# phylo42/IPK

Hardware: AMD Instinct MI355X
Metric: scored phylo-k-mers/sec (higher is better)
Workload: dtype f32

## Files before the change

ipk_amd/csrc/ipkgpu.hip:

```cpp
#include <cstring>
#include <hip/hip_runtime.h>
#include <rocprim/rocprim.hpp>

#include <algorithm>
#include <cmath>
#include <cstdarg>
#include <cstdio>
#include <cstring>
#include <new>
#include <string>
#include <type_traits>
#include <unordered_map>
#include <memory>
#include <vector>

#include "../../include/ipkgpu.h"
#include "dcla_device.hpp"
#include "kernels_score.hpp"
#include "kernels_quad.hpp"
#include "kernels_compact.hpp"
#include "kernels_keymajor.hpp"
#include "kernels_reduce_pipe.hpp"
#include "kernels_filter.hpp"
#include "kernels_dbfile.hpp"
// ... 59 lines not shown
    ipkgpu_comm* comm = nullptr;
    hipStream_t stream = nullptr;
    std::string err;
    int64_t workspace_bytes = 0;
    int64_t opt_variant = 0;
    int64_t opt_flags = 0;
    int64_t opt_kmc_pass = 0;
    int64_t opt_slice = 0;
    uint64_t sliced_windows = 0;
    int64_t opt_prefix_mats = 0;
    int64_t opt_wg_chunks2 = 0;
    int64_t opt_rounds = 0;
    int64_t opt_pool_limit = 0;
    int64_t opt_pool_chunks = 0;
    DevBuf table, best, ovfq, counts, offsets, goff, idx, branch, scan_sums, scan_boff, tmp_a, tmp_b, tmp_c;
    DevBuf pool, desc, gbcnt, gboff, gbcur, clist, gm, tile_next;
    DevBuf ptrs;
    DevBuf sp_bits, sp_pops, sp_rank, sp_c16;
    void* h_spill[2] = {nullptr, nullptr}; hipEvent_t ev_spill[2] = {nullptr, nullptr}; size_t h_spill_cap = 0;
    size_t held = 0, held_peak = 0;
    int64_t budget = 0;
    size_t refused_need = 0;
    DevBuf mask;
    bool mask_valid = false;
    uint64_t mask_words = 0;
    bool table_compressed = false;
    DevBuf rank, vaddr, ucnt, qpack, xstart, pcounts;
    DevBuf seq, pvals, pvaddr, mrank, cursnap;
    DevBuf cvals, coff, croom;
    bool comp_own_vals = false;
// ... 234 lines not shown
        *got = ctx->free_blocks[best].second;
        ctx->live_blocks[*out] = *got;
        ctx->cached_bytes -= *got;
        ctx->free_blocks.erase(ctx->free_blocks.begin() + best);
        return hipSuccess;
    }
    const hipError_t e = ctx_alloc(ctx, out, want_bytes);
    if (e == hipSuccess) *got = ctx->live_blocks[*out];
    return e;
}

static std::vector<DevBuf*> all_workspaces(ipkgpu_ctx* ctx)
{
    return {&ctx->table, &ctx->best, &ctx->ovfq, &ctx->counts, &ctx->offsets, &ctx->goff, &ctx->idx,
            &ctx->branch, &ctx->scan_sums, &ctx->scan_boff, &ctx->tmp_a, &ctx->tmp_b, &ctx->tmp_c,
            &ctx->pool, &ctx->desc, &ctx->gbcnt, &ctx->gboff, &ctx->gbcur, &ctx->clist, &ctx->gm, &ctx->tile_next, &ctx->mask,
            &ctx->rank, &ctx->vaddr, &ctx->ucnt, &ctx->qpack, &ctx->xstart, &ctx->pcounts, &ctx->ptrs,
            &ctx->cvals, &ctx->coff, &ctx->croom, &ctx->seq, &ctx->pvals, &ctx->pvaddr, &ctx->mrank, &ctx->cursnap,
            &ctx->sp_bits, &ctx->sp_pops, &ctx->sp_rank, &ctx->sp_c16,
            &ctx->place_seq, &ctx->place_off, &ctx->place_out, &ctx->place_tables, &ctx->place_small, &ctx->place_amb};
}

extern "C" {

uint32_t ipkgpu_bits_per_symbol(uint32_t sigma) { return sigma == 4 ? 2u : sigma == 20 ? 5u : 0u; }
uint32_t ipkgpu_max_k(uint32_t sigma) { return sigma == 4 ? 14u : sigma == 20 ? 6u : 0u; }
uint32_t ipkgpu_max_k_keyrange(uint32_t sigma) { return sigma == 4 ? 16u : ipkgpu_max_k(sigma); }
size_t ipkgpu_kmer_batch(uint32_t key, size_t n_ranges) { return n_ranges ? key % n_ranges : 0; }

float ipkgpu_log_threshold(float omega, uint32_t sigma, uint32_t k)
{
// ... 324 lines not shown
#ifndef IPK_QROWLANE
#define IPK_QROWLANE 0
#endif
template <int SIGMA, int K> constexpr bool quad_rowlane() { return K <= 10 ? IPK_QROWLANE != 0 : IPK_QROWLANE12 != 0; }
#ifndef IPK_QONEWIN12
#define IPK_QONEWIN12 1
#endif
template <int SIGMA, int K> constexpr bool quad_onewin() { return K >= 11 && IPK_QONEWIN12 != 0 && quad_rowlane<SIGMA, K>(); }
#ifndef IPK_PAIR6
#define IPK_PAIR6 1
#endif
template <int SIGMA, int K> constexpr PairLayout quad_layout()
{
    return IPK_PAIR6 != 0 && quad_ok<SIGMA, K>() && K <= 10 && !quad_rowlane<SIGMA, K>() ? PairLayout::PAIR6 : PairLayout::PAIR8;
}
template <int SIGMA, int K> size_t quad_lds()
{
    if constexpr (!quad_ok<SIGMA, K>()) return 0;
    else {
        constexpr int CAP = fast_cap<SIGMA, K>();
        constexpr uint32_t TBL = stream_tbl<SIGMA, K>();
        constexpr uint32_t NB = (uint32_t)((ipow(SIGMA, K) + TBL - 1) / TBL);
        return QuadTile<SIGMA, K, quad_tw<SIGMA, K>()>::HEAD_BYTES + (size_t)quad_nw<SIGMA, K>() * quad_wave_entries<SIGMA, K, CAP, quad_onewin<SIGMA, K>()>() * 8 +
               (size_t)quad_nw<SIGMA, K>() * NB * 8;
    }
}
template <int SIGMA, int K, bool COUNT_ONLY = false>
int launch_quad_pass1(ipkgpu_ctx* ctx, const StreamParams& sp, uint32_t n_wg, PairLayout layout)
{
    if constexpr (!quad_ok<SIGMA, K>()) { (void)sp; (void)n_wg; (void)layout; return fail(ctx, IPKGPU_ERR_INVALID, "quad kernel unsupported for this sigma/k"); }
    else {
        if (layout != quad_layout<SIGMA, K>()) return fail(ctx, IPKGPU_ERR_INVALID, "the pass' pool layout is not the quad kernel's");
        constexpr int CAP = fast_cap<SIGMA, K>();
        constexpr uint32_t TBL = stream_tbl<SIGMA, K>();
        constexpr int QNW = quad_nw<SIGMA, K>(), QTW = quad_tw<SIGMA, K>();
        const size_t lds = quad_lds<SIGMA, K>();
        auto kern = score_quad_kernel<SIGMA, K, CAP, QTW, QNW, TBL, COUNT_ONLY, quad_rowlane<SIGMA, K>(), quad_onewin<SIGMA, K>(), quad_layout<SIGMA, K>()>;
        if (lds > 64 * 1024)
            HIP_TRY(ctx, hipFuncSetAttribute(reinterpret_cast<const void*>(kern), hipFuncAttributeMaxDynamicSharedMemorySize, (int)lds));
        hipLaunchKernelGGL(kern, dim3(n_wg), dim3(QNW * 64), lds, ctx->stream, sp);
        HIP_TRY(ctx, hipGetLastError());
        return IPKGPU_OK;
    }
}

#ifndef IPK_XPNW
#define IPK_XPNW 11
#endif
#ifndef IPK_XPTW
#define IPK_XPTW 128
#endif
constexpr int XP_TW = IPK_XPTW;
// ... 123 lines not shown
            case 15 * 8 + 2: return f(int_c<4>{}, int_c<15>{}, int_c<13>{});
            case 16 * 8 + 2: return f(int_c<4>{}, int_c<16>{}, int_c<14>{});
            case 16 * 8 + 3: return f(int_c<4>{}, int_c<16>{}, int_c<13>{});
        }
    }
    return fail(ctx, IPKGPU_ERR_INVALID, "unsupported key range");
}

struct Geometry {
    uint32_t fast_cap = 0;
    uint32_t stream_nb = 0, stream_tbl = 0;
    uint32_t stream_nw = NW, stream_tw = TW;
    size_t stream_lds = 0;
    bool quad = false;
    uint32_t quad_nw = NW, quad_tw = TW;
    size_t quad_lds = 0;
    PairLayout quad_layout = PairLayout::PAIR8;
    uint32_t xp_nb = 0, xp_tbl = 0;
    size_t xp_lds = 0;
};

int fill_geometry(ipkgpu_ctx* ctx, uint32_t sigma, uint32_t k, uint32_t lead, Geometry& g)
{
    if (!lead)
        RC_TRY(with_sigma_k(ctx, sigma, k, [&](auto S_, auto K_) {
            g.fast_cap = fast_cap<S_, K_>();
            g.stream_nb = stream_nb<S_, K_>(); g.stream_tbl = stream_tbl<S_, K_>();
            g.stream_nw = stream_nw<S_, K_>(); g.stream_tw = stream_tw<S_, K_>(); g.stream_lds = stream_lds<S_, K_>();
            g.quad = quad_ok<S_, K_>();
            g.quad_nw = quad_nw<S_, K_>(); g.quad_tw = quad_tw<S_, K_>(); g.quad_lds = quad_lds<S_, K_>();
            g.quad_layout = quad_layout<S_, K_>();
            return IPKGPU_OK;
        }));
    return with_xp_shape(ctx, sigma, k, lead, [&](auto S_, auto K_, auto KK_) {
        g.xp_nb = xp_nb<S_, K_, KK_>(); g.xp_tbl = xp_tbl<S_, K_>(); g.xp_lds = xp_lds<S_, K_, KK_>();
        return IPKGPU_OK;
    });
}

#ifndef IPK_KMC_RUNS_DEFAULT
#define IPK_KMC_RUNS_DEFAULT 1
#endif
#ifndef IPK_KMC_PASS
#define IPK_KMC_PASS 256
#endif
#define KM_LAUNCH(KERN, CAPV, ...)                                                                                        \
// ... 486 lines not shown
        else if (cap < n_waves * NBK * SUB) {
            if (gb > 1) return IPKGPU_RETRY_SMALLER;
            return fail(ctx, IPKGPU_ERR_NOMEM, "the pair pool of ONE branch group does not fit device memory");
        }
        RC_TRY(ensure(ctx, ctx->pool, (cap + 1) * CHB));
        RC_TRY(ensure(ctx, ctx->desc, cap * 8));
        if (!forced) cap = std::min<uint64_t>(ctx->pool.cap / CHB - 1, ctx->desc.cap / 8);
        RC_TRY(ensure(ctx, ctx->gbcnt, 2 * n_gb * 4));
        uint32_t* const d_gbcur = ctx->gbcnt.as<uint32_t>() + n_gb;
        RC_TRY(ensure(ctx, ctx->gboff, (n_gb + 1) * 8));
        uint32_t* d_pool_next = small_at(ctx, SMALL_POOL_NEXT);
        uint32_t* d_pool_ovf = small_at(ctx, SMALL_POOL_OVF);
        const bool pre_ok = use_quad && n_waves * NBK + 1024 <= cap && !(ctx->opt_flags & 32);
        const uint32_t pre_chunks = pre_ok ? (uint32_t)(n_waves * NBK) : 0u;
        uint32_t* d_tile_next = nullptr;
        if (use_quad && !(ctx->opt_flags & 128) && ((uint64_t)nb * s_tiles_per_mat >= 4ull * gb * S || (ctx->opt_flags & 256))) {
            RC_TRY(ensure(ctx, ctx->tile_next, (size_t)gb * 4));
            d_tile_next = ctx->tile_next.as<uint32_t>();
        }
        hipLaunchKernelGGL(small_reset_kernel, dim3((std::max<uint32_t>(gb, SMALL_XP_TOO_BIG / 4) + 255) / 256), dim3(256), 0, ctx->stream,
                           reinterpret_cast<uint32_t*>(ctx->small), pre_chunks, d_tile_next, gb, S);
        HIP_TRY(ctx, hipGetLastError());
        HIP_TRY(ctx, hipMemsetAsync(ctx->desc.p, 0, cap * 8, ctx->stream));

        StreamParams sp;
        sp.logp = logp_dev; sp.best = ctx->best.as<float>();
        sp.gm_off = ctx->gm.as<uint32_t>(); sp.gm_list = ctx->gm.as<uint32_t>() + gb + 1;
        sp.sites = pl.sites; sp.nwin = pl.nwin; sp.tiles_per_mat = s_tiles_per_mat; sp.S = S;
        sp.eps = pl.eps;
        sp.pool = ctx->pool.as<uint2>(); sp.pool_cap = (uint32_t)cap; sp.pool_next = d_pool_next;
        sp.desc = ctx->desc.as<unsigned long long>(); sp.pool_ovf = d_pool_ovf;
        sp.emitted = p.emitted; sp.ovf_queue = p.ovf_queue; sp.ovf_count = p.ovf_count; sp.mat_slot = p.mat_slot;
        sp.flags = (uint32_t)(ctx->opt_flags);
        sp.pre_chunks = pre_chunks;
        sp.tile_next = d_tile_next;
        std::unique_ptr<Stopwatch> sw_own(new Stopwatch(ctx->stream, &ctx->events));
        Stopwatch& sw = *sw_own;
        const int ev_a = sw.mark();
        RC_TRY(pass1(sp, n_wg, false));
        const int ev_b = sw.mark();
        const bool spec = ctx->spec_skip_wait && !s_compress && !(ctx->opt_flags & 64);
        uint32_t n_ovf = 0;
        uint32_t h[2] = {0, 0};
        if (!spec) {
            HIP_TRY(ctx, hipMemcpyAsync(ctx->h_rb, ctx->small, SMALL_BYTES, hipMemcpyDeviceToHost, ctx->stream));
            HIP_TRY(ctx, hipStreamSynchronize(ctx->stream));
            n_ovf = ctx->h_rb[SMALL_OVF_COUNT / 4]; h[0] = ctx->h_rb[SMALL_POOL_NEXT / 4]; h[1] = ctx->h_rb[SMALL_POOL_OVF / 4];
        }
        const bool ovf_in_pool = n_ovf > 0 && ((uint64_t)n_ovf * IPK_OVF_POOL_RATIO >= windows || s_compress) && pool_ovf_ok;
        if (ovf_in_pool) {
// ... 1469 lines not shown
extern "C" {

int ipkgpu_get_option(const ipkgpu_ctx* ctx, const char* name, int64_t* value)
{
    if (!ctx || !name || !value) return IPKGPU_ERR_INVALID;
    if (!strcmp(name, "workspace_bytes")) { *value = ctx->workspace_bytes; return IPKGPU_OK; }
    if (!strcmp(name, "device_budget_bytes")) { *value = ctx->budget; return IPKGPU_OK; }
    if (!strcmp(name, "last_refused_bytes")) { *value = (int64_t)ctx->refused_need; return IPKGPU_OK; }
    if (!strcmp(name, "slice_long_lists")) { *value = ctx->opt_slice; return IPKGPU_OK; }
    if (!strcmp(name, "db_load_chunk_bytes")) { *value = ctx->opt_load_chunk; return IPKGPU_OK; }
    if (!strcmp(name, "place_batch_queries")) { *value = ctx->opt_place_batch; return IPKGPU_OK; }
    if (!strcmp(name, "place_lds_branches")) { *value = ctx->opt_place_lds; return IPKGPU_OK; }
    if (!strcmp(name, "debug_sliced_windows")) { *value = (int64_t)ctx->sliced_windows; return IPKGPU_OK; }
    if (!strcmp(name, "debug_count_pass_pairs")) { *value = (int64_t)ctx->count_pass_pairs; return IPKGPU_OK; }
    if (!strcmp(name, "debug_count_pass_queued")) { *value = (int64_t)ctx->count_pass_queued; return IPKGPU_OK; }
    if (!strcmp(name, "debug_pool_bytes")) { *value = (int64_t)ctx->pool.cap; return IPKGPU_OK; }
    return IPKGPU_ERR_INVALID;
}

int ipkgpu_mem_stats(ipkgpu_ctx* ctx, uint64_t* held, uint64_t* held_peak, int reset_peak)
{
    if (!ctx) return IPKGPU_ERR_INVALID;
    if (held) *held = ctx->held;
    if (held_peak) *held_peak = ctx->held_peak;
    if (reset_peak) ctx->held_peak = ctx->held;
    return IPKGPU_OK;
}

int ipkgpu_parts_spill(ipkgpu_ctx* ctx, ipkgpu_parts* parts, const char* dir, uint32_t piece, uint64_t* bytes_written)
{
// ... 201 lines not shown
```

ipk_amd/csrc/kernels_quad.hpp:

```cpp
#pragma once
#include "kernels_score.hpp"

namespace ipkgpu {

struct QuadNode { int J, H, TH, OFF; uint32_t F, CMUL; };
struct QuadStep { int H, A, B; };

template <int SIGMA, int K>
struct QuadGeo {
    using D = HalvesDD<SIGMA, K>;
    static constexpr int HL = D::HL, HR = D::HR, LA = D::LA, LB = D::LB, RA = D::RA, RB = D::RB;
    static constexpr bool OK = SIGMA == 4 && D::OK && LA >= 2 && LA <= 3 && LB >= 2 && LB <= 3 && RA >= 2 && RA <= 3 && RB >= 2 && RB <= 3;
    static constexpr uint32_t FLA = D::FLA, FLB = D::FLB, FRA = D::FRA, FRB = D::FRB;
    static constexpr uint32_t mulR = ipow(SIGMA, K - K / 2);
    static constexpr uint32_t CW = FLA + FLB + FRA + FRB;
    static constexpr int th_n(int h) { return h == 2 ? 3 : 5; }
    static constexpr int TH0 = 2, TH1 = TH0 + th_n(LA), TH2 = TH1 + th_n(LB), TH3 = TH2 + th_n(RA);
    static constexpr int TH_F = TH3 + th_n(RB);
    static constexpr int PADW = 1;
    static constexpr QuadNode node(int n)
    {
        return n == 0 ? QuadNode{0, LA, TH0, 0, FLA, 1u}
             : n == 1 ? QuadNode{LA, LB, TH1, (int)FLA, FLB, mulR}
             : n == 2 ? QuadNode{HL, RA, TH2, (int)(FLA + FLB), FRA, 1u}
                      : QuadNode{HL + RA, RB, TH3, (int)(FLA + FLB + FRA), FRB, 1u};
    }
    static constexpr int count_h(int h) { int c = 0; for (int n = 0; n < 4; ++n) c += node(n).H == h; return c; }
    static constexpr int nth_h(int h, int i) { for (int n = 0; n < 4; ++n) if (node(n).H == h) { if (i == 0) return n; --i; } return -1; }
    static constexpr int NS2 = (count_h(2) + 1) / 2, NS3 = (count_h(3) + 1) / 2, NSTEPS = NS2 + NS3;
    static constexpr QuadStep step(int s)
    {
        return s < NS2 ? QuadStep{2, nth_h(2, 2 * s), nth_h(2, 2 * s + 1)} : QuadStep{3, nth_h(3, 2 * (s - NS2)), nth_h(3, 2 * (s - NS2) + 1)};
    }
    static constexpr int step_of(int n) { for (int s = 0; s < NSTEPS; ++s) if (step(s).A == n || step(s).B == n) return s; return -1; }
    static constexpr int slot_of(int n) { return step(step_of(n)).B == n ? 1 : 0; }
    static constexpr int NS1 = (count_h(2) > 0 ? 1 : 0) + (count_h(3) > 0 ? 1 : 0);
    static constexpr int step1_h(int s) { return (s == 0 && count_h(2) > 0) ? 2 : 3; }
    static constexpr int step1_node(int s, int slot) { return nth_h(step1_h(s), slot); }
    static constexpr int step1_of(int n) { return node(n).H == 2 ? 0 : (count_h(2) > 0 ? 1 : 0); }
    static constexpr int slot1_of(int n) { int c = 0; for (int m = 0; m < n; ++m) c += node(m).H == node(n).H; return c; }
};

template <int SIGMA, int K, int TW>
struct QuadTile {
    static constexpr int TC = TW + K - 1 + QuadGeo<SIGMA, K>::PADW;
    static constexpr int COLS_F = TC * SIGMA;
    static constexpr int BEST_F = ((TC + 1 + 3) / 4) * 4;
    static constexpr int TH_FLOATS = (((TW + QuadGeo<SIGMA, K>::PADW) * QuadGeo<SIGMA, K>::TH_F + 3) / 4) * 4;
    static constexpr int HEAD_BYTES = (COLS_F + BEST_F + TH_FLOATS) * 4;
};

template <int SIGMA, int K, int CAP, bool ONEWIN = false>
constexpr uint32_t quad_wave_entries()
{
    using Q = QuadGeo<SIGMA, K>;
    return (ONEWIN ? 1 : 2) * Q::CW + Geo<SIGMA, Q::HL, CAP>::CAPH + Geo<SIGMA, Q::HR, CAP>::CAPH;
}

template <int J, int H>
__device__ __forceinline__ void quad_node_thresholds(const float* bs, float e, float* out)
{
    out[0] = e;
    if constexpr (H == 2) {
        out[1] = e - (bs[J + 2] - bs[J + 1]);
        out[2] = e - (bs[J + 1] - bs[J]);
// ... 30 lines not shown
__device__ __forceinline__ uint2 lds_entry(uint32_t base, uint32_t j)
{
    typedef const u32x2_t __attribute__((address_space(3)))* lds_pair_ptr;
    uint32_t a;
    asm("v_lshl_add_u32 %0, %1, 3, %2" : "=v"(a) : "v"(j), "s"(base));
    const u32x2_t v = *(lds_pair_ptr)(uintptr_t)a;
    return make_uint2(v.x, v.y);
}
__device__ __forceinline__ uint32_t bcnt_add(uint32_t x, uint32_t acc)
{
    uint32_t r;
    asm("v_bcnt_u32_b32 %0, %1, %2" : "=v"(r) : "v"(x), "v"(acc));
    return r;
}

template <int H>
__device__ __forceinline__ void quad_step(const float* ca, const float* cb, const float* ci, uint64_t vmask, const float* th, uint32_t list,
                                          uint32_t sh16, uint32_t lt16, uint32_t lt16w, uint32_t code16, uint32_t cmul, uint32_t& count)
{
    const float e = th[0];
    if constexpr (H == 2) {
        const float sl = ca[0], sr = cb[0];
        const float s = sl + sr;
        const bool c1 = sl > th[1], c2 = sr > th[2], c3 = s > e;
        const uint64_t m = vmask & ballot64(c1) & ballot64(c2) & ballot64(c3);
        const uint32_t x = (uint32_t)(m >> sh16);
        lds_put8_lanes(lshl3_add((uint32_t)__popc(x & lt16), list), code16, __float_as_uint(s), m);
        count = (uint32_t)__popc(x & 0xFFFFu);
    } else {
        const float sj = ca[0], sl2 = cb[0];
        const float s2 = sj + sl2;
        const bool d1 = sj > th[3], d2 = sl2 > th[4], d3 = s2 > th[2];
        const uint64_t mp = vmask & ballot64(d1) & ballot64(d2) & ballot64(d3);
        float s[4]; uint64_t m[4]; uint32_t x[4];
#pragma unroll
        for (int i = 0; i < 4; ++i) {
            const float si = ci[i];
            s[i] = si + s2;
            const bool c1 = si > th[1], c2 = s[i] > e;
            m[i] = mp & ballot64(c1) & ballot64(c2);
            x[i] = (uint32_t)(m[i] >> sh16);
        }
        const uint32_t y01 = __builtin_amdgcn_perm(x[1], x[0], 0x05040100u);
        const uint32_t y23 = __builtin_amdgcn_perm(x[3], x[2], 0x05040100u);
        const uint32_t n01 = (uint32_t)__popc(y01);
        const uint32_t pos[4] = {(uint32_t)__popc(x[0] & lt16), (uint32_t)__popc(y01 & lt16w), bcnt_add(x[2] & lt16, n01), bcnt_add(y23 & lt16w, n01)};
#pragma unroll
        for (int i = 0; i < 4; ++i) lds_put8_lanes(lshl3_add(pos[i], list), __umul24(cmul, (uint32_t)i * 16u) + code16, __float_as_uint(s[i]), m[i]);
        count = bcnt_add(y23, n01);
    }
}

__device__ __forceinline__ void pool_store(uint2* wave_base, uint32_t byte_off, uint2 val)
{
    const unsigned long long data = ((unsigned long long)val.y << 32) | val.x;
    asm volatile("global_store_dwordx2 %0, %1, %2" : : "v"(byte_off), "v"(data), "s"(wave_base) : "memory");
}
__device__ __forceinline__ void pool_store_lanes(uint2* wave_base, uint32_t byte_off, uint2 val, uint64_t mask)
{
    const unsigned long long data = ((unsigned long long)val.y << 32) | val.x;
    IPK_ASSERT_FULL_EXEC();
    asm volatile("s_mov_b64 exec, %3\n\tglobal_store_dwordx2 %0, %1, %2\n\ts_mov_b64 exec, -1"
                 : : "v"(byte_off), "v"(data), "s"(wave_base), "s"(mask) : "memory");
// ... 32 lines not shown
__device__ __forceinline__ uint64_t pool_store_inside6(uint2* wave_base, uint32_t off4, uint32_t off2, uint2 val, uint32_t v, uint64_t pass, uint32_t CH)
{
    static_assert(SLOT_PLANE < 4096, "the slot plane's offset must fit the store's immediate field");
    uint64_t outside;
    IPK_ASSERT_FULL_EXEC();
    asm volatile("s_mov_b64 exec, %7\n\t"
                 "v_cmpx_gt_u32_e32 vcc, %8, %6\n\t"
                 "global_store_dword %1, %3, %5\n\t"
                 "global_store_short %2, %4, %5 offset:%9\n\t"
                 "s_andn2_b64 %0, %7, exec\n\t"
                 "s_mov_b64 exec, -1"
                 : "=&s"(outside) : "v"(off4), "v"(off2), "v"(val.y), "v"(val.x), "s"(wave_base), "v"(v), "s"(pass), "s"(CH), "n"(SLOT_PLANE)
                 : "memory", "vcc");
    return outside;
}

constexpr uint32_t QUAD_SPAN_BYTES_LOG2 = 32;
constexpr uint32_t QUAD_SPAN_TEST = 8;

__device__ __forceinline__ uint32_t div_small(float x_plus_half, float rn) { return (uint32_t)(x_plus_half * rn); }

template <uint32_t NB, uint32_t CH, uint32_t PAIR_BYTES = 8u>
struct RowAppender {
    static constexpr uint32_t NONE = 0xFFFFFFFFu;
    static constexpr uint32_t CHUNK_BYTES = CH * PAIR_BYTES;
    static constexpr uint32_t SPAN_CHUNKS = (uint32_t)((1ull << QUAD_SPAN_BYTES_LOG2) / CHUNK_BYTES);
    const StreamParams& p;
    unsigned long long* st;
    uint32_t g;
    uint32_t chunk_next = 0, chunk_end = 0;
// ... 151 lines not shown
    uint32_t n = 0;
    for (uint32_t i0 = 0; i0 < na; i0 += rps) {
        const uint2 a = ap[i0];
        const float s = __uint_as_float(a.y) + by;
        const bool live = lane < min(rps, na - i0) * nb, c = s > eps;
        const uint64_t m = ballot64(live) & ballot64(c);
        const uint32_t cnt = (uint32_t)__popcll(m);
        if (n + cnt > cap) return LIST_OVERFLOW;
        if (live && c) (out + n)[mbcnt(m)] = make_uint2(a.x * MUL + b.x, __float_as_uint(s));
        n += cnt;
    }
    return n;
}

template <int SIGMA, int K, int CAP, int TW, int NW, uint32_t TBL, bool COUNT_ONLY = false, bool ROWLANE = false, bool ONEWIN = false,
          PairLayout LAYOUT = PairLayout::PAIR8>
__global__ __launch_bounds__(NW * 64) void score_quad_kernel(StreamParams p)
{
    extern __shared__ __align__(16) unsigned char smem[];
    using Q = QuadGeo<SIGMA, K>;
    using QT = QuadTile<SIGMA, K, TW>;
    static_assert(Q::OK, "quad kernel: DNA k = 8..12");
    constexpr uint32_t T = ipow(SIGMA, K);
    constexpr uint32_t NB = (T + TBL - 1) / TBL;
    constexpr uint32_t CH = chunk_pairs<TBL>();
    constexpr uint32_t mulR = Q::mulR;
    static_assert(TBL % mulR == 0, "a row of the final join must stay inside one bucket");
    using CL = ChunkLayout<TBL, LAYOUT>;
    static_assert(!ROWLANE || LAYOUT == PairLayout::PAIR8, "the row-per-lane join writes 8-byte pairs");
    constexpr bool P6 = LAYOUT == PairLayout::PAIR6;
    constexpr uint32_t CAPL = Geo<SIGMA, Q::HL, CAP>::CAPH, CAPR = Geo<SIGMA, Q::HR, CAP>::CAPH;
    constexpr uint32_t WS = quad_wave_entries<SIGMA, K, CAP, ONEWIN>();
    constexpr uint32_t WPW = ONEWIN ? 1u : 2u;
    constexpr int NST = ONEWIN ? Q::NS1 : Q::NSTEPS;
    float* cols = reinterpret_cast<float*>(smem);
    float* best = cols + QT::COLS_F;
    float* thr = best + QT::BEST_F;
    uint2* scratch_all = reinterpret_cast<uint2*>(smem + QT::HEAD_BYTES);
    unsigned long long* state_all = reinterpret_cast<unsigned long long*>(scratch_all + (size_t)NW * WS);

    const uint32_t lane = lane_id();
    const uint32_t wave = (uint32_t)__builtin_amdgcn_readfirstlane((int)(threadIdx.x >> 6));
    const uint32_t g = blockIdx.x / p.S, seg = blockIdx.x - g * p.S;
    const uint32_t m0 = p.gm_off[g], nm = p.gm_off[g + 1] - m0;
    const uint32_t total_tiles = nm * p.tiles_per_mat;
    const uint32_t t_lo = (uint32_t)(((uint64_t)total_tiles * seg) / p.S);
    const uint32_t t_hi = (uint32_t)(((uint64_t)total_tiles * (seg + 1)) / p.S);

    uint2* child = scratch_all + (size_t)wave * WS;
    uint2* lp = child + WPW * Q::CW;
    uint2* rp = lp + CAPL;
    constexpr uint32_t LP_OFF = WPW * Q::CW * 8u, RP_OFF = LP_OFF + CAPL * 8u;
    const uint32_t child_a = lds_addr(child);
    using Appender = std::conditional_t<ROWLANE, LaneAppender<NB, CH>, RowAppender<NB, CH, CL::PAIR_BYTES>>;
    Appender app{p, state_all + (size_t)wave * NB, g};
    app.init(blockIdx.x * NW + wave);
    unsigned long long emitted = 0;
// ... 23 lines not shown
                if (n >= 0 && slot == (uint32_t)sl) nd = Q::node(n);
            }
            j4 = (uint32_t)nd.J * 4u; tho = (uint32_t)nd.TH; off = (uint32_t)nd.OFF; st_cmul[s] = nd.CMUL;
            ST_ON[s] = on;
        } else {
            const QuadStep qs = Q::step(s);
            const QuadNode na = Q::node(qs.A), nb = qs.B >= 0 ? Q::node(qs.B) : none;
            j4 = sb ? (uint32_t)nb.J * 4u : (uint32_t)na.J * 4u;
            tho = sb ? (uint32_t)nb.TH : (uint32_t)na.TH;
            off = (sb ? (uint32_t)nb.OFF : (uint32_t)na.OFF) + half * Q::CW;
            st_cmul[s] = sb ? nb.CMUL : na.CMUL;
            ST_ON[s] = qs.B >= 0 ? ~0ull : 0x0000FFFF0000FFFFull;
        }
        st_code[s] = l16 * st_cmul[s];
        const int H = ONEWIN ? Q::step1_h(s) : Q::step(s < Q::NSTEPS ? s : 0).H;
        const float* c0 = cols + (wave * WPW + half) * 4u + j4;
        st_ci[s] = c0;
        st_ca[s] = c0 + (H == 2 ? 0u : 4u) + (l16 >> 2);
        st_cb[s] = c0 + (H == 2 ? 4u : 8u) + (l16 & 3u);
        st_thp[s] = thr + (wave * WPW + half) * (uint32_t)Q::TH_F + tho;
        st_list[s] = child_a + off * 8u;
        asm("" : "+v"(st_list[s]));
    }

    __shared__ uint32_t sh_tile;
    const bool draw = p.tile_next != nullptr;
    uint32_t t = t_lo, t_end = t_hi;
    if (draw) { t = seg; t_end = total_tiles; }
    while (t < t_end) {
        const uint32_t q = t / p.tiles_per_mat, tile = t - q * p.tiles_per_mat;
        const uint32_t mat = p.gm_list[m0 + q];
        const uint32_t t0 = tile * TW;
        const uint32_t nw = min((uint32_t)TW, p.nwin - t0);
        const uint32_t ncol = nw + K - 1;
        __syncthreads();
        uint32_t t_drawn = 0;
        if (draw && threadIdx.x == 0) t_drawn = atomicAdd(&p.tile_next[g], 1u);
        {
            const float4* src = reinterpret_cast<const float4*>(p.logp + ((size_t)mat * p.sites + t0) * SIGMA);
            float4* dst = reinterpret_cast<float4*>(cols);
            const uint32_t n4 = ncol * (SIGMA / 4);
            for (uint32_t i = threadIdx.x; i < n4; i += NW * 64) dst[i] = src[i];
            const float* bsrc = p.best + (size_t)mat * (p.sites + 1) + t0;
            for (uint32_t i = threadIdx.x; i <= ncol; i += NW * 64) best[i] = bsrc[i];
        }
        if (draw && threadIdx.x == 0) sh_tile = t_drawn;
        __syncthreads();
        for (uint32_t w = threadIdx.x; w < nw; w += NW * 64) {
            const float* bs = best + w;
            float* o = thr + w * Q::TH_F;
            const float eps_l = eps - (bs[K] - bs[Q::HL]);
            const float eps_r = eps - (bs[Q::HL] - bs[0]);
            o[0] = eps_l; o[1] = eps_r;
            quad_node_thresholds<0, Q::LA>(bs, eps_l - (bs[Q::HL] - bs[Q::LA]), o + Q::node(0).TH);
            quad_node_thresholds<Q::LA, Q::LB>(bs, eps_l - (bs[Q::LA] - bs[0]), o + Q::node(1).TH);
            quad_node_thresholds<Q::HL, Q::RA>(bs, eps_r - (bs[K] - bs[Q::HL + Q::RA]), o + Q::node(2).TH);
            quad_node_thresholds<Q::HL + Q::RA, Q::RB>(bs, eps_r - (bs[Q::HL + Q::RA] - bs[Q::HL]), o + Q::node(3).TH);
        }
        __syncthreads();

        const uint32_t npair = (nw + WPW - 1) / WPW;
        for (uint32_t pr = wave; pr < npair; pr += NW) {
            const uint32_t wq = pr * WPW;
            const uint32_t wo = wq - wave * WPW;
            const uint64_t wmask = ONEWIN || wq + 1 < nw ? ~0ull : 0xFFFFFFFFull;
            uint32_t counts[3] = {0, 0, 0};
            wave_lds_sync();
            auto run_step = [&](auto S) {
                constexpr int s = decltype(S)::value;
                if constexpr (s < NST) {
                    constexpr int H = ONEWIN ? Q::step1_h(s) : Q::step(s < Q::NSTEPS ? s : 0).H;
                    const uint32_t co = wo * 4u, to = wo * (uint32_t)Q::TH_F;
                    const float* ca = st_ca[s] + co;
                    quad_step<H>(ca, CB_FROM_CA ? ca + cb_ca : st_cb[s] + co, st_ci[s] + co, wmask & ST_ON[s], st_thp[s] + to, st_list[s], sh16, lt16, lt16w,
                                 st_code[s], st_cmul[s], counts[s]);
                }
            };
            run_step(std::integral_constant<int, 0>{});
            run_step(std::integral_constant<int, 1>{});
            run_step(std::integral_constant<int, 2>{});
            wave_lds_sync();
            const uint32_t nwp = min(WPW, nw - wq);

#pragma unroll 1
            for (uint32_t gw = 0; gw < nwp; ++gw) {
                const uint32_t w = wq + gw;
                constexpr int so0 = ONEWIN ? Q::step1_of(0) : Q::step_of(0), so1 = ONEWIN ? Q::step1_of(1) : Q::step_of(1);
                constexpr int so2 = ONEWIN ? Q::step1_of(2) : Q::step_of(2), so3 = ONEWIN ? Q::step1_of(3) : Q::step_of(3);
// ... 37 lines not shown
                           : (uint32_t)__builtin_amdgcn_readfirstlane((int)(tr <= 64 ? half_join_single<Q::FRB, RP_OFF>(ra, rb, nrb, tr, eps_r, child_a, lane, lane_h)
                                                                                      : half_join_rows<Q::FRB>(ra, nra, rb, nrb, eps_r, rp, CAPR, lane, lane_h)));
                    } else {
                    if (!keep_l)
                        nL = (uint32_t)__builtin_amdgcn_readfirstlane((int)join_to_list(la + ia, min(sla, nla - ia), lb, nlb, eps_l, Q::FLB * mulR, lp, CAPL));
                    if constexpr (SLICE) {
                        if (nL == LIST_OVERFLOW) { sla = SAFE_L; continue; }
                    }
                    nR = nL == LIST_OVERFLOW || nL == 0 ? nL : (uint32_t)__builtin_amdgcn_readfirstlane((int)join_to_list(ra + ir, min(sra, nra - ir), rb, nrb, eps_r, Q::FRB, rp, CAPR));
                    }
                    if constexpr (SLICE) {
                        if (nR == LIST_OVERFLOW) { sra = SAFE_R; keep_l = true; continue; }
                    } else if (nL == LIST_OVERFLOW || nR == LIST_OVERFLOW) {
                        if (lane == 0) {
                            const uint32_t qi = atomicAdd(p.ovf_count, 1u);
                            p.ovf_queue[qi] = ((unsigned long long)mat << 32) | (unsigned long long)(t0 + w);
                        }
                        __builtin_amdgcn_wave_barrier();
                        break;
                    }
                }
                if (nL != 0 && nR != 0) {
                wave_lds_sync();
                if (p.flags & 4u) emitted += nL + nR;
                else
                if constexpr (ROWLANE) {
                    constexpr uint32_t CB = 64;
                    static_assert(CB <= CH, "row-per-lane join: a run must fit a chunk");
                    for (uint32_t ib = 0; ib < nL; ib += 64) {
                        const uint2 a = lp[ib + lane];
// ... 161 lines not shown
                    using I3 = std::integral_constant<int, 3>;
                    for (; i0 + 3 * rps <= nL; i0 += 3 * rps) trip(I3{}, std::true_type{}, i0);
                    for (; i0 + 2 * rps <= nL; i0 += 2 * rps) trip(I2{}, std::true_type{}, i0);
                    if (i0 + rps < nL) trip(I2{}, std::false_type{}, i0);
                    else if (i0 < nL) trip(I1{}, std::false_type{}, i0);
                }
                }
                if (!SLICE || one_step) break;
                ir += sra;
                if (nL != 0 && ir < nra) { keep_l = true; continue; }
                ir = 0; keep_l = false; ia += sla;
                if (ia >= nla) break;
                }
            }
        }
        t = draw ? sh_tile : t + 1;
    }
    if (!count_only) app.close();
    if (lane == 0 && emitted) atomicAdd(p.emitted, emitted);
}

}
```

ipk_amd/csrc/kernels_score.hpp:

```cpp
#pragma once
#include <type_traits>
#include "dcla_device.hpp"

namespace ipkgpu {


template <int SIGMA, int M>
__global__ __launch_bounds__(256) void prefix_max_kernel(const float* __restrict__ logp, uint32_t n_mats, uint32_t sites,
                                                         float* __restrict__ best)
{
    constexpr int CH = 2048 / M;
    constexpr int ROW = CH + 4;
    static_assert(M == 1 || M == 2 || M == 4 || M == 8, "matrices per workgroup");
    __shared__ __align__(16) float cmbuf[2][M][ROW];
    const uint32_t mat0 = blockIdx.x * M;
    const uint32_t mv = min((uint32_t)M, n_mats - mat0);
    const bool chain = threadIdx.x < mv;
    const uint32_t my = mat0 + (chain ? threadIdx.x : 0u);
    float* b = best + (size_t)my * (sites + 1);
    if (chain) b[0] = 0.0f;
    float carry = 0.0f;
    auto maxima = [&](uint32_t c0, float (*cmw)[ROW], uint32_t t0, uint32_t nt) {
        const uint32_t n = min((uint32_t)CH, sites - c0);
        for (uint32_t mm = 0; mm < mv; ++mm) {
// ... 416 lines not shown
    const uint32_t* gm_list;
    uint32_t sites, nwin, tiles_per_mat, S;
    float eps;
    uint32_t slice_lists = 0;
    uint2* pool;
    uint32_t pool_cap;
    uint32_t* pool_next;
    unsigned long long* desc;
    uint32_t* pool_ovf;
    unsigned long long* emitted;
    unsigned long long* ovf_queue;
    uint32_t* ovf_count;
    const uint32_t* mat_slot;
    uint32_t flags;
    uint32_t pre_chunks;
    uint32_t* tile_next = nullptr;
    uint32_t* big_ovf = nullptr;
};

__device__ __constant__ uint32_t RCP16[65] = {
    0, 65536, 32768, 21846, 16384, 13108, 10923, 9363, 8192, 7282, 6554, 5958, 5462, 5042, 4682, 4370, 4096,
    3856, 3641, 3450, 3277, 3121, 2979, 2850, 2731, 2622, 2521, 2428, 2341, 2260, 2185, 2115, 2048,
    1986, 1928, 1873, 1821, 1772, 1725, 1681, 1639, 1599, 1561, 1525, 1490, 1457, 1425, 1395, 1366,
    1338, 1311, 1286, 1261, 1237, 1214, 1192, 1171, 1150, 1130, 1111, 1093, 1075, 1058, 1041, 1024};

template <int SIGMA, int K>
struct HalvesDD {
    static constexpr int HL = K / 2, HR = K - K / 2;
    static constexpr int LA = HL / 2, LB = HL - LA, RA = HR / 2, RB = HR - RA;
    static constexpr bool OK = ipow(SIGMA, HL) > 64 && ipow(SIGMA, LB) <= 64 && ipow(SIGMA, RB) <= 64;
// ... 1260 lines not shown
```

Measured before the change: 144.6 billion.

## Give each wave its own window strip with prefetched loads in quad kernel

For k<=10 non-rowlane quad paths, each wave now independently draws small strips of SW windows, keeps per-wave column, best and threshold areas in LDS, and prefetches the next strip into registers while scoring the current one. This removes the workgroup-wide __syncthreads tile loads, and each wave draws its next strip with a single lane-63 atomic. Compile-time step offsets also let list addresses become immediates. It adds an optional wait-time probe, but strips are small, so per-strip overhead and load-balance heuristics change.

```diff
diff --git a/ipk_amd/csrc/ipkgpu.hip b/ipk_amd/csrc/ipkgpu.hip
--- a/ipk_amd/csrc/ipkgpu.hip
+++ b/ipk_amd/csrc/ipkgpu.hip
@@ -97,6 +97,7 @@
     int64_t opt_pool_limit = 0;
     int64_t opt_pool_chunks = 0;
     DevBuf table, best, ovfq, counts, offsets, goff, idx, branch, scan_sums, scan_boff, tmp_a, tmp_b, tmp_c;
+    DevBuf qwaits;
     DevBuf pool, desc, gbcnt, gboff, gbcur, clist, gm, tile_next;
     DevBuf ptrs;
     DevBuf sp_bits, sp_pops, sp_rank, sp_c16;
@@ -361,7 +362,7 @@
 {
     return {&ctx->table, &ctx->best, &ctx->ovfq, &ctx->counts, &ctx->offsets, &ctx->goff, &ctx->idx,
             &ctx->branch, &ctx->scan_sums, &ctx->scan_boff, &ctx->tmp_a, &ctx->tmp_b, &ctx->tmp_c,
-            &ctx->pool, &ctx->desc, &ctx->gbcnt, &ctx->gboff, &ctx->gbcur, &ctx->clist, &ctx->gm, &ctx->tile_next, &ctx->mask,
+            &ctx->pool, &ctx->desc, &ctx->gbcnt, &ctx->gboff, &ctx->gbcur, &ctx->clist, &ctx->gm, &ctx->tile_next, &ctx->qwaits, &ctx->mask,
             &ctx->rank, &ctx->vaddr, &ctx->ucnt, &ctx->qpack, &ctx->xstart, &ctx->pcounts, &ctx->ptrs,
             &ctx->cvals, &ctx->coff, &ctx->croom, &ctx->seq, &ctx->pvals, &ctx->pvaddr, &ctx->mrank, &ctx->cursnap,
             &ctx->sp_bits, &ctx->sp_pops, &ctx->sp_rank, &ctx->sp_c16,
@@ -716,6 +717,13 @@
 {
     return IPK_PAIR6 != 0 && quad_ok<SIGMA, K>() && K <= 10 && !quad_rowlane<SIGMA, K>() ? PairLayout::PAIR6 : PairLayout::PAIR8;
 }
+#ifndef IPK_QSTRIPS
+#define IPK_QSTRIPS 1
+#endif
+#ifndef IPK_QSW
+#define IPK_QSW 8
+#endif
+template <int SIGMA, int K> constexpr bool quad_strips() { return IPK_QSTRIPS != 0 && quad_ok<SIGMA, K>() && K <= 10 && !quad_rowlane<SIGMA, K>() && !quad_onewin<SIGMA, K>(); }
 template <int SIGMA, int K> size_t quad_lds()
 {
     if constexpr (!quad_ok<SIGMA, K>()) return 0;
@@ -723,7 +731,9 @@
         constexpr int CAP = fast_cap<SIGMA, K>();
         constexpr uint32_t TBL = stream_tbl<SIGMA, K>();
         constexpr uint32_t NB = (uint32_t)((ipow(SIGMA, K) + TBL - 1) / TBL);
-        return QuadTile<SIGMA, K, quad_tw<SIGMA, K>()>::HEAD_BYTES + (size_t)quad_nw<SIGMA, K>() * quad_wave_entries<SIGMA, K, CAP, quad_onewin<SIGMA, K>()>() * 8 +
+        constexpr size_t head = quad_head_bytes<SIGMA, K, quad_tw<SIGMA, K>(), quad_nw<SIGMA, K>(), quad_strips<SIGMA, K>(), IPK_QSW>();
+        static_assert(head <= (size_t)QuadTile<SIGMA, K, quad_tw<SIGMA, K>()>::HEAD_BYTES, "the strip areas must fit the tile head they replace");
+        return head + (size_t)quad_nw<SIGMA, K>() * quad_wave_entries<SIGMA, K, CAP, quad_onewin<SIGMA, K>()>() * 8 +
                (size_t)quad_nw<SIGMA, K>() * NB * 8;
     }
 }
@@ -737,7 +747,8 @@
         constexpr uint32_t TBL = stream_tbl<SIGMA, K>();
         constexpr int QNW = quad_nw<SIGMA, K>(), QTW = quad_tw<SIGMA, K>();
         const size_t lds = quad_lds<SIGMA, K>();
-        auto kern = score_quad_kernel<SIGMA, K, CAP, QTW, QNW, TBL, COUNT_ONLY, quad_rowlane<SIGMA, K>(), quad_onewin<SIGMA, K>(), quad_layout<SIGMA, K>()>;
+        auto kern = score_quad_kernel<SIGMA, K, CAP, QTW, QNW, TBL, COUNT_ONLY, quad_rowlane<SIGMA, K>(), quad_onewin<SIGMA, K>(), quad_layout<SIGMA, K>(),
+                                      quad_strips<SIGMA, K>(), IPK_QSW>;
         if (lds > 64 * 1024)
             HIP_TRY(ctx, hipFuncSetAttribute(reinterpret_cast<const void*>(kern), hipFuncAttributeMaxDynamicSharedMemorySize, (int)lds));
         hipLaunchKernelGGL(kern, dim3(n_wg), dim3(QNW * 64), lds, ctx->stream, sp);
@@ -891,6 +902,7 @@
     size_t stream_lds = 0;
     bool quad = false;
     uint32_t quad_nw = NW, quad_tw = TW;
+    uint32_t quad_strip_w = 0;
     size_t quad_lds = 0;
     PairLayout quad_layout = PairLayout::PAIR8;
     uint32_t xp_nb = 0, xp_tbl = 0;
@@ -907,6 +919,7 @@
             g.quad = quad_ok<S_, K_>();
             g.quad_nw = quad_nw<S_, K_>(); g.quad_tw = quad_tw<S_, K_>(); g.quad_lds = quad_lds<S_, K_>();
             g.quad_layout = quad_layout<S_, K_>();
+            g.quad_strip_w = quad_strips<S_, K_>() ? (uint32_t)IPK_QSW : 0u;
             return IPKGPU_OK;
         }));
     return with_xp_shape(ctx, sigma, k, lead, [&](auto S_, auto K_, auto KK_) {
@@ -1423,12 +1436,15 @@
         const bool pre_ok = use_quad && n_waves * NBK + 1024 <= cap && !(ctx->opt_flags & 32);
         const uint32_t pre_chunks = pre_ok ? (uint32_t)(n_waves * NBK) : 0u;
         uint32_t* d_tile_next = nullptr;
-        if (use_quad && !(ctx->opt_flags & 128) && ((uint64_t)nb * s_tiles_per_mat >= 4ull * gb * S || (ctx->opt_flags & 256))) {
+        const uint32_t QSW = use_quad ? pl.geo.quad_strip_w : 0u;
+        const uint64_t work_units = QSW ? (uint64_t)nb * ((pl.nwin + QSW - 1) / QSW) * QSW : (uint64_t)nb * s_tiles_per_mat * STW;
+        const uint32_t first_drawn = QSW ? 2u * S * SNW : S;
+        if (use_quad && !(ctx->opt_flags & 128) && (work_units >= 4ull * STW * gb * S || (ctx->opt_flags & 256))) {
             RC_TRY(ensure(ctx, ctx->tile_next, (size_t)gb * 4));
             d_tile_next = ctx->tile_next.as<uint32_t>();
         }
         hipLaunchKernelGGL(small_reset_kernel, dim3((std::max<uint32_t>(gb, SMALL_XP_TOO_BIG / 4) + 255) / 256), dim3(256), 0, ctx->stream,
-                           reinterpret_cast<uint32_t*>(ctx->small), pre_chunks, d_tile_next, gb, S);
+                           reinterpret_cast<uint32_t*>(ctx->small), pre_chunks, d_tile_next, gb, first_drawn);
         HIP_TRY(ctx, hipGetLastError());
         HIP_TRY(ctx, hipMemsetAsync(ctx->desc.p, 0, cap * 8, ctx->stream));
 
@@ -1443,6 +1459,14 @@
         sp.flags = (uint32_t)(ctx->opt_flags);
         sp.pre_chunks = pre_chunks;
         sp.tile_next = d_tile_next;
+#ifdef IPK_QWAITS
+        if (use_quad) {
+            const bool fresh = ctx->qwaits.p == nullptr;
+            RC_TRY(ensure(ctx, ctx->qwaits, 6 * 8));
+            if (fresh) HIP_TRY(ctx, hipMemsetAsync(ctx->qwaits.p, 0, 6 * 8, ctx->stream));
+            sp.waits = ctx->qwaits.as<unsigned long long>();
+        }
+#endif
         std::unique_ptr<Stopwatch> sw_own(new Stopwatch(ctx->stream, &ctx->events));
         Stopwatch& sw = *sw_own;
         const int ev_a = sw.mark();
@@ -2942,6 +2966,18 @@
     if (!strcmp(name, "debug_sliced_windows")) { *value = (int64_t)ctx->sliced_windows; return IPKGPU_OK; }
     if (!strcmp(name, "debug_count_pass_pairs")) { *value = (int64_t)ctx->count_pass_pairs; return IPKGPU_OK; }
     if (!strcmp(name, "debug_count_pass_queued")) { *value = (int64_t)ctx->count_pass_queued; return IPKGPU_OK; }
+    if (!strcmp(name, "quad_strip_windows")) { *value = quad_strips<4, 10>() ? (int64_t)IPK_QSW : 0; return IPKGPU_OK; }
+#ifdef IPK_QWAITS
+    if (!strncmp(name, "debug_quad_waits_", 17) && name[17] >= '0' && name[17] <= '5' && !name[18]) {
+        unsigned long long v = 0;
+        if (ctx->qwaits.p) {
+            if (hipStreamSynchronize(ctx->stream) != hipSuccess) return IPKGPU_ERR_INVALID;
+            if (hipMemcpy(&v, ctx->qwaits.as<unsigned long long>() + (name[17] - '0'), 8, hipMemcpyDeviceToHost) != hipSuccess) return IPKGPU_ERR_INVALID;
+        }
+        *value = (int64_t)v;
+        return IPKGPU_OK;
+    }
+#endif
     if (!strcmp(name, "debug_pool_bytes")) { *value = (int64_t)ctx->pool.cap; return IPKGPU_OK; }
     return IPKGPU_ERR_INVALID;
 }
diff --git a/ipk_amd/csrc/kernels_quad.hpp b/ipk_amd/csrc/kernels_quad.hpp
--- a/ipk_amd/csrc/kernels_quad.hpp
+++ b/ipk_amd/csrc/kernels_quad.hpp
@@ -34,6 +34,15 @@
     }
     static constexpr int step_of(int n) { for (int s = 0; s < NSTEPS; ++s) if (step(s).A == n || step(s).B == n) return s; return -1; }
     static constexpr int slot_of(int n) { return step(step_of(n)).B == n ? 1 : 0; }
+    static constexpr int th_delta(int s) { return node(step(s).A).TH - node(step(0).A).TH; }
+    static constexpr int off_delta(int s) { return node(step(s).A).OFF - node(step(0).A).OFF; }
+    static constexpr bool delta_ok(int s)
+    {
+        if (th_delta(s) < 0 || off_delta(s) < 0) return false;
+        if (step(s).B < 0) return true;
+        return step(0).B >= 0 && node(step(s).B).TH - node(step(0).B).TH == th_delta(s) && node(step(s).B).OFF - node(step(0).B).OFF == off_delta(s);
+    }
+    static constexpr bool deltas_ok() { for (int s = 1; s < NSTEPS; ++s) if (!delta_ok(s)) return false; return true; }
     static constexpr int NS1 = (count_h(2) > 0 ? 1 : 0) + (count_h(3) > 0 ? 1 : 0);
     static constexpr int step1_h(int s) { return (s == 0 && count_h(2) > 0) ? 2 : 3; }
     static constexpr int step1_node(int s, int slot) { return nth_h(step1_h(s), slot); }
@@ -49,6 +58,24 @@
     static constexpr int TH_FLOATS = (((TW + QuadGeo<SIGMA, K>::PADW) * QuadGeo<SIGMA, K>::TH_F + 3) / 4) * 4;
     static constexpr int HEAD_BYTES = (COLS_F + BEST_F + TH_FLOATS) * 4;
 };
+
+template <int SIGMA, int K, int SW>
+struct QuadStrip {
+    static_assert(SW % 2 == 0 && SW >= 2 && SW * 4 <= 64, "a strip: whole window pairs, one lane per (window, node) for the thresholds");
+    static constexpr int SC = SW + K - 1 + QuadGeo<SIGMA, K>::PADW;
+    static constexpr int COLS_F = SC * SIGMA;
+    static constexpr int BEST_F = ((SW + K + 3) / 4) * 4;
+    static constexpr int TH_FLOATS = ((SW * QuadGeo<SIGMA, K>::TH_F + 3) / 4) * 4;
+    static constexpr int WAVE_F = COLS_F + BEST_F + TH_FLOATS;
+    static constexpr int WAVE_BYTES = WAVE_F * 4;
+};
+
+template <int SIGMA, int K, int TW, int NW, bool STRIPS, int SW>
+constexpr int quad_head_bytes()
+{
+    if constexpr (STRIPS) return NW * QuadStrip<SIGMA, K, SW>::WAVE_BYTES;
+    else return QuadTile<SIGMA, K, TW>::HEAD_BYTES;
+}
 
 template <int SIGMA, int K, int CAP, bool ONEWIN = false>
 constexpr uint32_t quad_wave_entries()
@@ -109,7 +136,7 @@
     return r;
 }
 
-template <int H>
+template <int H, uint32_t LIST_IMM = 0>
 __device__ __forceinline__ void quad_step(const float* ca, const float* cb, const float* ci, uint64_t vmask, const float* th, uint32_t list,
                                           uint32_t sh16, uint32_t lt16, uint32_t lt16w, uint32_t code16, uint32_t cmul, uint32_t& count)
 {
@@ -120,7 +147,7 @@
         const bool c1 = sl > th[1], c2 = sr > th[2], c3 = s > e;
         const uint64_t m = vmask & ballot64(c1) & ballot64(c2) & ballot64(c3);
         const uint32_t x = (uint32_t)(m >> sh16);
-        lds_put8_lanes(lshl3_add((uint32_t)__popc(x & lt16), list), code16, __float_as_uint(s), m);
+        lds_put8_lanes<LIST_IMM>(lshl3_add((uint32_t)__popc(x & lt16), list), code16, __float_as_uint(s), m);
         count = (uint32_t)__popc(x & 0xFFFFu);
     } else {
         const float sj = ca[0], sl2 = cb[0];
@@ -141,7 +168,7 @@
         const uint32_t n01 = (uint32_t)__popc(y01);
         const uint32_t pos[4] = {(uint32_t)__popc(x[0] & lt16), (uint32_t)__popc(y01 & lt16w), bcnt_add(x[2] & lt16, n01), bcnt_add(y23 & lt16w, n01)};
 #pragma unroll
-        for (int i = 0; i < 4; ++i) lds_put8_lanes(lshl3_add(pos[i], list), __umul24(cmul, (uint32_t)i * 16u) + code16, __float_as_uint(s[i]), m[i]);
+        for (int i = 0; i < 4; ++i) lds_put8_lanes<LIST_IMM>(lshl3_add(pos[i], list), __umul24(cmul, (uint32_t)i * 16u) + code16, __float_as_uint(s[i]), m[i]);
         count = bcnt_add(y23, n01);
     }
 }
@@ -204,6 +231,21 @@
                  : "memory", "vcc");
     return outside;
 }
+
+#ifdef IPK_QWAITS
+#define IPK_QW(i) do { const long long qw_n = wall_clock64(); qw_t[i] += (unsigned long long)(qw_n - qw_last); qw_last = qw_n; } while (0)
+#else
+#define IPK_QW(i) ((void)0)
+#endif
+
+__device__ __forceinline__ void draw_into_lane63(uint32_t& reg, uint32_t* counter)
+{
+    const uint32_t zero = 0u, one = 1u;
+    IPK_ASSERT_FULL_EXEC();
+    asm volatile("s_mov_b64 exec, %4\n\tglobal_atomic_add %0, %1, %2, %3 sc0\n\ts_mov_b64 exec, -1"
+                 : "=v"(reg) : "v"(zero), "v"(one), "s"(counter), "s"(0x8000000000000000ull) : "memory");
+}
+__device__ __forceinline__ void wait_vmem() { asm volatile("s_waitcnt vmcnt(0)" : : : "memory"); }
 
 constexpr uint32_t QUAD_SPAN_BYTES_LOG2 = 32;
 constexpr uint32_t QUAD_SPAN_TEST = 8;
@@ -385,13 +427,15 @@
 }
 
 template <int SIGMA, int K, int CAP, int TW, int NW, uint32_t TBL, bool COUNT_ONLY = false, bool ROWLANE = false, bool ONEWIN = false,
-          PairLayout LAYOUT = PairLayout::PAIR8>
+          PairLayout LAYOUT = PairLayout::PAIR8, bool STRIPS = false, int SW = 8>
 __global__ __launch_bounds__(NW * 64) void score_quad_kernel(StreamParams p)
 {
     extern __shared__ __align__(16) unsigned char smem[];
     using Q = QuadGeo<SIGMA, K>;
     using QT = QuadTile<SIGMA, K, TW>;
+    using QS = QuadStrip<SIGMA, K, SW>;
     static_assert(Q::OK, "quad kernel: DNA k = 8..12");
+    static_assert(!STRIPS || (!ONEWIN && !ROWLANE), "strips: the two-window child steps and the candidate-per-lane join");
     constexpr uint32_t T = ipow(SIGMA, K);
     constexpr uint32_t NB = (T + TBL - 1) / TBL;
     constexpr uint32_t CH = chunk_pairs<TBL>();
@@ -404,14 +448,14 @@
     constexpr uint32_t WS = quad_wave_entries<SIGMA, K, CAP, ONEWIN>();
     constexpr uint32_t WPW = ONEWIN ? 1u : 2u;
     constexpr int NST = ONEWIN ? Q::NS1 : Q::NSTEPS;
-    float* cols = reinterpret_cast<float*>(smem);
-    float* best = cols + QT::COLS_F;
-    float* thr = best + QT::BEST_F;
-    uint2* scratch_all = reinterpret_cast<uint2*>(smem + QT::HEAD_BYTES);
-    unsigned long long* state_all = reinterpret_cast<unsigned long long*>(scratch_all + (size_t)NW * WS);
-
     const uint32_t lane = lane_id();
     const uint32_t wave = (uint32_t)__builtin_amdgcn_readfirstlane((int)(threadIdx.x >> 6));
+    float* cols = reinterpret_cast<float*>(smem) + (STRIPS ? wave * (uint32_t)QS::WAVE_F : 0u);
+    float* best = cols + (STRIPS ? QS::COLS_F : QT::COLS_F);
+    float* thr = best + (STRIPS ? QS::BEST_F : QT::BEST_F);
+    uint2* scratch_all = reinterpret_cast<uint2*>(smem + quad_head_bytes<SIGMA, K, TW, NW, STRIPS, SW>());
+    unsigned long long* state_all = reinterpret_cast<unsigned long long*>(scratch_all + (size_t)NW * WS);
+
     const uint32_t g = blockIdx.x / p.S, seg = blockIdx.x - g * p.S;
     const uint32_t m0 = p.gm_off[g], nm = p.gm_off[g + 1] - m0;
     const uint32_t total_tiles = nm * p.tiles_per_mat;
@@ -465,11 +509,12 @@
         }
         st_code[s] = l16 * st_cmul[s];
         const int H = ONEWIN ? Q::step1_h(s) : Q::step(s < Q::NSTEPS ? s : 0).H;
-        const float* c0 = cols + (wave * WPW + half) * 4u + j4;
+        const uint32_t w_first = (STRIPS ? 0u : wave * WPW) + half;
+        const float* c0 = cols + w_first * 4u + j4;
         st_ci[s] = c0;
         st_ca[s] = c0 + (H == 2 ? 0u : 4u) + (l16 >> 2);
         st_cb[s] = c0 + (H == 2 ? 4u : 8u) + (l16 & 3u);
-        st_thp[s] = thr + (wave * WPW + half) * (uint32_t)Q::TH_F + tho;
+        st_thp[s] = thr + w_first * (uint32_t)Q::TH_F + tho;
         st_list[s] = child_a + off * 8u;
         asm("" : "+v"(st_list[s]));
     }
@@ -478,14 +523,115 @@
     const bool draw = p.tile_next != nullptr;
     uint32_t t = t_lo, t_end = t_hi;
     if (draw) { t = seg; t_end = total_tiles; }
+
+    const uint32_t spm = STRIPS ? (p.nwin + (uint32_t)SW - 1u) / (uint32_t)SW : 1u;
+    const uint32_t spm_rcp = spm > 1u ? (uint32_t)(0x100000000ull / spm) : 0xFFFFFFFFu;
+    constexpr uint32_t PF_B = 16;
+    static_assert(!STRIPS || (SIGMA * (SW + K - 1) <= 64 + PF_B && PF_B + SW + K < 63), "a strip in flight: two registers");
+    uint32_t t_n1 = 0, s_nw = 0;
+    uint32_t c_q = 0xFFFFFFFFu, c_mat = 0;
+    float pf_c; uint32_t pf_x;
+    if constexpr (STRIPS) asm volatile("" : "=v"(pf_c), "=v"(pf_x));
+    auto strip_locate = [&](uint32_t s, uint32_t& q, uint32_t& t0_) {
+        q = __umulhi(s, spm_rcp);
+        uint32_t r = s - q * spm;
+        if (r >= spm) { ++q; r -= spm; }
+        t0_ = r * (uint32_t)SW;
+    };
+    auto strip_windows = [&](uint32_t s) {
+        uint32_t q, t0_;
+        strip_locate(s, q, t0_);
+        return min((uint32_t)SW, p.nwin - t0_);
+    };
+    auto strip_load = [&](uint32_t s) {
+        uint32_t q, t0_;
+        strip_locate(s, q, t0_);
+        if (q != c_q) { c_q = q; c_mat = (uint32_t)__builtin_amdgcn_readfirstlane((int)p.gm_list[m0 + q]); }
+        const uint32_t mat_ = c_mat;
+        const uint32_t ncol = min((uint32_t)SW, p.nwin - t0_) + K - 1;
+        const float* src = p.logp + ((size_t)mat_ * p.sites + t0_) * SIGMA;
+        const float* bsrc = p.best + (size_t)mat_ * (p.sites + 1) + t0_;
+        if (lane < ncol * SIGMA) pf_c = src[lane];
+        if (lane + 64u < ncol * SIGMA) pf_x = __float_as_uint(src[lane + 64u]);
+        if (lane >= PF_B && lane <= ncol + PF_B) pf_x = __float_as_uint((bsrc - PF_B)[lane]);
+    };
+    auto strip_put = [&](uint32_t nw_) {
+        const uint32_t ncol = nw_ + K - 1;
+        wave_lds_sync();
+        if (lane < ncol * SIGMA) cols[lane] = pf_c;
+        if (lane + 64u < ncol * SIGMA) cols[lane + 64u] = __uint_as_float(pf_x);
+        if (lane >= PF_B && lane <= ncol + PF_B) (best - PF_B)[lane] = __uint_as_float(pf_x);
+        wave_lds_sync();
+        uint32_t ln = lane;
+        asm volatile("" : "+v"(ln));
+        if (ln < (uint32_t)SW * 4u) {
+            const uint32_t tw = ln % (uint32_t)SW, nd = ln / (uint32_t)SW;
+            auto pack = [](int n) {
+                const QuadNode q = Q::node(n);
+                const uint32_t n1 = n == 0 ? Q::HL : n == 1 ? Q::LA : n == 2 ? K : Q::HL + Q::RA;
+                const uint32_t n2 = n == 0 ? Q::LA : n == 1 ? 0 : n == 2 ? Q::HL + Q::RA : Q::HL;
+                return n1 | n2 << 4 | (uint32_t)q.J << 8 | (uint32_t)q.TH << 12 | (q.H == 3 ? 1u << 17 : 0u);
+            };
+            const uint32_t pk = nd == 0 ? pack(0) : nd == 1 ? pack(1) : nd == 2 ? pack(2) : pack(3);
+            const bool left = nd < 2, h3 = (pk >> 17) != 0;
+            const float* bs = best + tw;
+            const float bK = bs[K], bH = bs[Q::HL], bZ = bs[0];
+            const float eps_l = eps - (bK - bH);
+            const float eps_r = eps - (bH - bZ);
+            const float eh = left ? eps_l : eps_r;
+            const float e = eh - (bs[pk & 15u] - bs[(pk >> 4) & 15u]);
+            const float* bj = bs + ((pk >> 8) & 15u);
+            const float b0 = bj[0], b1 = bj[1], b2 = bj[2], b3 = bj[3];
+            float* o = thr + tw * (uint32_t)Q::TH_F;
+            o[left ? 0 : 1] = eh;
+            o += (pk >> 12) & 31u;
+            const float o2 = e - (b1 - b0);
+            o[0] = e;
+            o[1] = e - ((h3 ? b3 : b2) - b1);
+            o[2] = o2;
+            if (h3) {
+                o[3] = o2 - (b3 - b2);
+                o[4] = o2 - (b2 - b1);
+            }
+        }
+        wave_lds_sync();
+    };
+#ifdef IPK_QWAITS
+    unsigned long long qw_t[5] = {0, 0, 0, 0, 0};
+    long long qw_last = wall_clock64();
+#endif
+    if constexpr (STRIPS) {
+        const uint32_t total_strips = nm * spm, n_waves = p.S * NW, wg = seg * NW + wave;
+        if (draw) { t = wg; t_n1 = wg + n_waves; t_end = total_strips; }
+        else {
+            t = (uint32_t)(((uint64_t)total_strips * wg) / n_waves);
+            t_end = (uint32_t)(((uint64_t)total_strips * (wg + 1)) / n_waves);
+            t_n1 = t + 1;
+        }
+        if (t < t_end) {
+            s_nw = strip_windows(t);
+            strip_load(t);
+            strip_put(s_nw);
+        }
+    }
+    IPK_QW(4);
     while (t < t_end) {
+      uint32_t mat = 0, t0 = 0, nw;
+      [[maybe_unused]] uint32_t t_drawn = 0;
+      if constexpr (STRIPS) {
+        nw = s_nw;
+        if (draw) draw_into_lane63(pf_x, p.tile_next + g);
+        else asm volatile("" : "=v"(pf_x));
+        if (t_n1 < t_end) strip_load(t_n1);
+        IPK_QW(1);
+      } else {
         const uint32_t q = t / p.tiles_per_mat, tile = t - q * p.tiles_per_mat;
-        const uint32_t mat = p.gm_list[m0 + q];
-        const uint32_t t0 = tile * TW;
-        const uint32_t nw = min((uint32_t)TW, p.nwin - t0);
+        mat = p.gm_list[m0 + q];
+        t0 = tile * TW;
+        nw = min((uint32_t)TW, p.nwin - t0);
         const uint32_t ncol = nw + K - 1;
         __syncthreads();
-        uint32_t t_drawn = 0;
+        IPK_QW(0);
         if (draw && threadIdx.x == 0) t_drawn = atomicAdd(&p.tile_next[g], 1u);
         {
             const float4* src = reinterpret_cast<const float4*>(p.logp + ((size_t)mat * p.sites + t0) * SIGMA);
@@ -497,6 +643,7 @@
         }
         if (draw && threadIdx.x == 0) sh_tile = t_drawn;
         __syncthreads();
+        IPK_QW(1);
         for (uint32_t w = threadIdx.x; w < nw; w += NW * 64) {
             const float* bs = best + w;
             float* o = thr + w * Q::TH_F;
@@ -509,11 +656,13 @@
             quad_node_thresholds<Q::HL + Q::RA, Q::RB>(bs, eps_r - (bs[Q::HL + Q::RA] - bs[Q::HL]), o + Q::node(3).TH);
         }
         __syncthreads();
+        IPK_QW(2);
+      }
 
         const uint32_t npair = (nw + WPW - 1) / WPW;
-        for (uint32_t pr = wave; pr < npair; pr += NW) {
+        for (uint32_t pr = STRIPS ? 0u : wave; pr < npair; pr += STRIPS ? 1u : (uint32_t)NW) {
             const uint32_t wq = pr * WPW;
-            const uint32_t wo = wq - wave * WPW;
+            const uint32_t wo = STRIPS ? wq : wq - wave * WPW;
             const uint64_t wmask = ONEWIN || wq + 1 < nw ? ~0ull : 0xFFFFFFFFull;
             uint32_t counts[3] = {0, 0, 0};
             wave_lds_sync();
@@ -523,6 +672,10 @@
                     constexpr int H = ONEWIN ? Q::step1_h(s) : Q::step(s < Q::NSTEPS ? s : 0).H;
                     const uint32_t co = wo * 4u, to = wo * (uint32_t)Q::TH_F;
                     const float* ca = st_ca[s] + co;
+                    if constexpr (STRIPS && Q::deltas_ok())
+                        quad_step<H, (uint32_t)Q::off_delta(s < Q::NSTEPS ? s : 0) * 8u>(ca, CB_FROM_CA ? ca + cb_ca : st_cb[s] + co, st_ci[s] + co, wmask & ST_ON[s],
+                                     st_thp[0] + Q::th_delta(s < Q::NSTEPS ? s : 0) + to, st_list[0], sh16, lt16, lt16w, st_code[s], st_cmul[s], counts[s]);
+                    else
                     quad_step<H>(ca, CB_FROM_CA ? ca + cb_ca : st_cb[s] + co, st_ci[s] + co, wmask & ST_ON[s], st_thp[s] + to, st_list[s], sh16, lt16, lt16w,
                                  st_code[s], st_cmul[s], counts[s]);
                 }
@@ -590,6 +743,11 @@
                     } else if (nL == LIST_OVERFLOW || nR == LIST_OVERFLOW) {
                         if (lane == 0) {
                             const uint32_t qi = atomicAdd(p.ovf_count, 1u);
+                            if constexpr (STRIPS) {
+                                uint32_t q;
+                                strip_locate(t, q, t0);
+                                mat = p.gm_list[m0 + q];
+                            }
                             p.ovf_queue[qi] = ((unsigned long long)mat << 32) | (unsigned long long)(t0 + w);
                         }
                         __builtin_amdgcn_wave_barrier();
@@ -781,9 +939,27 @@
                 }
             }
         }
+        IPK_QW(3);
+        if constexpr (STRIPS) {
+            t = t_n1;
+            wait_vmem();
+            t_n1 = draw ? (uint32_t)__builtin_amdgcn_readlane((int)pf_x, 63) : t_n1 + 1u;
+            if (t < t_end) {
+                s_nw = strip_windows(t);
+                strip_put(s_nw);
+            }
+            IPK_QW(2);
+        } else
         t = draw ? sh_tile : t + 1;
     }
     if (!count_only) app.close();
+#ifdef IPK_QWAITS
+    IPK_QW(4);
+    if (lane == 0 && p.waits) {
+        for (int i = 0; i < 5; ++i) atomicAdd(&p.waits[i], qw_t[i]);
+        atomicAdd(&p.waits[5], 1ull);
+    }
+#endif
     if (lane == 0 && emitted) atomicAdd(p.emitted, emitted);
 }
 
diff --git a/ipk_amd/csrc/kernels_score.hpp b/ipk_amd/csrc/kernels_score.hpp
--- a/ipk_amd/csrc/kernels_score.hpp
+++ b/ipk_amd/csrc/kernels_score.hpp
@@ -454,6 +454,9 @@
     const uint32_t* mat_slot;
     uint32_t flags;
     uint32_t pre_chunks;
+#ifdef IPK_QWAITS
+    unsigned long long* waits = nullptr;
+#endif
     uint32_t* tile_next = nullptr;
     uint32_t* big_ovf = nullptr;
 };
```

After: 145.6 billion, median of 6. Within noise of the previous version (+0.7%).
